# houkensjtu/taichi-2d-vof

Measured on AMD Instinct MI355X. Metric: cell-updates/sec (whole node), 4096x4096 fp64 dam-break, higher is better.
Workload: dtype f64; 1 GPU; 4096x4096 -ic 1 f64, dt 4e-06, 10 Jacobi sweeps/step, single strip; nx=4096, ny=4096, jacobi_iters=10, exchange=none, tm_choice=1, step_schedule=k_tm batch graphs (k_transport + the next step's k_momentum as one kernel), handle_warm_steps=19

## Files before the change

### taichi-2d-vof_amd/csrc/kernels/common.h

```cpp
#pragma once
#include "../vof2d_device.h"

namespace vof {

#ifdef VOF_WAVE_TIMES
__device__ unsigned long long* vof_wave_times = nullptr;
__device__ int vof_wave_kid = -1;
__device__ unsigned int vof_wave_cap = 0;
struct WaveTimer {
  unsigned long long t0, c0, wait;
  unsigned int wave;
  bool on;
  __device__ __forceinline__ WaveTimer(int kid) {
    on = vof_wave_times != nullptr && vof_wave_kid == kid;
    wave = blockIdx.x * (blockDim.x >> 6) + (threadIdx.x >> 6);
    t0 = on ? wall_clock64() : 0ull;
    c0 = on ? __builtin_readcyclecounter() : 0ull;
    wait = 0ull;
  }
  __device__ __forceinline__ void barrier() {
    if (on) {
      const unsigned long long t = __builtin_readcyclecounter();
      __syncthreads();
      wait += __builtin_readcyclecounter() - t;
    } else {
      __syncthreads();
    }
  }
  __device__ __forceinline__ ~WaveTimer() {
    if (on && (threadIdx.x & 63) == 0 && wave < vof_wave_cap) {
      vof_wave_times[2 * wave] = t0;
      vof_wave_times[2 * wave + 1] = wall_clock64();
      vof_wave_times[2 * vof_wave_cap + 2 * wave] = wait;
      vof_wave_times[2 * vof_wave_cap + 2 * wave + 1] = __builtin_readcyclecounter() - c0;
    }
  }
};
#else
struct WaveTimer {
  __device__ __forceinline__ WaveTimer(int) {}
  __device__ __forceinline__ void barrier() { __syncthreads(); }
};
#endif
#ifdef VOF_SHORTCUT_STATS
__device__ unsigned long long vof_stats[16];
#define VOF_STAT(k) do { if ((threadIdx.x & 63) == 0) atomicAdd(&vof::vof_stats[k], 1ull); } while (0)
#else
#define VOF_STAT(k) do { } while (0)
#endif
enum : int { WT_MOMENTUM = 0, WT_JACOBI_TB = 3, WT_FCT_X = 5, WT_FCT_Y = 6, WT_JACOBI = 2, WT_TRANSPORT = 12, WT_JACOBI_PAIR = 13, WT_TM = 14 };
enum : int {
  ABL_FIXED_ROW = 1,
  ABL_NO_STORE = 2,
  ABL_PRIO0 = 4,
  ABL_PRIO1 = 8,
  ABL_IDLE1 = 16,
  ABL_PASS0 = 32,
  ABL_NO_UPRED = 64,
  ABL_NO_VPRED = 128
};
template <typename T, int V>
struct Row {
  T l;
  T c[V];
  T r;
};

template <typename T, int V>
__device__ __forceinline__ void load_c(T (&c)[V], const T* __restrict__ p) {
  Pack<T, V> k = *reinterpret_cast<const Pack<T, V>*>(p);
#pragma unroll
  for (int q = 0; q < V; ++q) c[q] = k.v[q];
}
template <typename T, int V>
__device__ __forceinline__ void load_row(Row<T, V>& w, const T* __restrict__ p) {
  load_c<T, V>(w.c, p);
  w.l = p[-1];
  w.r = p[V];
}
template <typename T, int V>
__device__ __forceinline__ void load_c_nt(T (&c)[V], const T* __restrict__ p) {
  typedef T vec_t __attribute__((ext_vector_type(V)));
  vec_t k = __builtin_nontemporal_load(reinterpret_cast<const vec_t*>(p));
#pragma unroll
  for (int q = 0; q < V; ++q) c[q] = k[q];
}
template <typename T, int V>
__device__ __forceinline__ void store_c_nt(T* __restrict__ p, const T (&c)[V], int j0, int jlo, int jhi) {
  typedef T vec_t __attribute__((ext_vector_type(V)));
  if (j0 >= jlo && j0 + V - 1 <= jhi) {
    vec_t k;
#pragma unroll
    for (int q = 0; q < V; ++q) k[q] = c[q];
    __builtin_nontemporal_store(k, reinterpret_cast<vec_t*>(p));
  } else {
#pragma unroll
    for (int q = 0; q < V; ++q)
      if (j0 + q >= jlo && j0 + q <= jhi) p[q] = c[q];
  }
}
template <typename T, int V>
__device__ __forceinline__ void store_c(T* __restrict__ p, const T (&c)[V], int j0, int jlo, int jhi) {
  if (j0 >= jlo && j0 + V - 1 <= jhi) {
    Pack<T, V> k;
#pragma unroll
    for (int q = 0; q < V; ++q) k.v[q] = c[q];
    *reinterpret_cast<Pack<T, V>*>(p) = k;
  } else {
#pragma unroll
    for (int q = 0; q < V; ++q)
      if (j0 + q >= jlo && j0 + q <= jhi) p[q] = c[q];
  }
}
template <typename T, int V>
__device__ __forceinline__ void load_s(T (&c)[V], const T* __restrict__ p) { load_c_nt<T, V>(c, p); }
template <typename T, int V>
__device__ __forceinline__ void store_s(T* __restrict__ p, const T (&c)[V], int j0, int jlo, int jhi) {
  store_c_nt<T, V>(p, c, j0, jlo, jhi);
}
constexpr int kBufSkip = (int)0x80000000;
template <typename T>
__device__ __forceinline__ T* wave_uniform(T* p) {
  const unsigned long long v = (unsigned long long)p;
  const unsigned lo = __builtin_amdgcn_readfirstlane((unsigned)v), hi = __builtin_amdgcn_readfirstlane((unsigned)(v >> 32));
  return (T*)(((unsigned long long)hi << 32) | lo);
}
template <typename T, int V>
__device__ __forceinline__ void store_buf_nt(const T* base, int lane_off_bytes, int row_off_bytes, const T (&c)[V]) {
  static_assert(sizeof(T) * V == 16 || sizeof(T) * V == 8, "one b128 / b64 store per lane");
  row_off_bytes = __builtin_amdgcn_readfirstlane(row_off_bytes);
  lane_off_bytes += row_off_bytes;
  asm volatile("" : "+v"(lane_off_bytes));
  row_off_bytes = 0;
  const __amdgpu_buffer_rsrc_t r = __builtin_amdgcn_make_buffer_rsrc(wave_uniform(const_cast<T*>(base)), 0, kBufSkip, 0x00020000);
  typedef T vec_t __attribute__((ext_vector_type(V)));
  vec_t k;
#pragma unroll
  for (int q = 0; q < V; ++q) k[q] = c[q];
  if constexpr (sizeof(T) * V == 16) {
    typedef unsigned int u4 __attribute__((ext_vector_type(4)));
    __builtin_amdgcn_raw_buffer_store_b128(__builtin_bit_cast(u4, k), r, lane_off_bytes, row_off_bytes, 2 );
  } else {
    typedef unsigned int u2 __attribute__((ext_vector_type(2)));
    __builtin_amdgcn_raw_buffer_store_b64(__builtin_bit_cast(u2, k), r, lane_off_bytes, row_off_bytes, 2 );
  }
}
template <typename T, int V>
__device__ __forceinline__ void load_buf(T (&c)[V], const T* base, int lane_off_bytes, int row_off_bytes, bool nt) {
  static_assert(sizeof(T) * V == 16 || sizeof(T) * V == 8, "one b128 / b64 load per lane");
  row_off_bytes = __builtin_amdgcn_readfirstlane(row_off_bytes);
  const __amdgpu_buffer_rsrc_t r = __builtin_amdgcn_make_buffer_rsrc(wave_uniform(const_cast<T*>(base)), 0, kBufSkip, 0x00020000);
  typedef T vec_t __attribute__((ext_vector_type(V)));
  vec_t k;
  if constexpr (sizeof(T) * V == 16) {
    typedef unsigned int u4 __attribute__((ext_vector_type(4)));
    const u4 w = nt ? __builtin_amdgcn_raw_buffer_load_b128(r, lane_off_bytes, row_off_bytes, 2) : __builtin_amdgcn_raw_buffer_load_b128(r, lane_off_bytes, row_off_bytes, 0);
    k = __builtin_bit_cast(vec_t, w);
  } else {
    typedef unsigned int u2 __attribute__((ext_vector_type(2)));
    const u2 w = nt ? __builtin_amdgcn_raw_buffer_load_b64(r, lane_off_bytes, row_off_bytes, 2) : __builtin_amdgcn_raw_buffer_load_b64(r, lane_off_bytes, row_off_bytes, 0);
    k = __builtin_bit_cast(vec_t, w);
  }
#pragma unroll
  for (int q = 0; q < V; ++q) c[q] = k[q];
}
template <typename T, int V>
__device__ __forceinline__ T left_of(const Row<T, V>& w, int q) { return q == 0 ? w.l : w.c[q - 1]; }
template <typename T, int V>
__device__ __forceinline__ T right_of(const Row<T, V>& w, int q) { return q == V - 1 ? w.r : w.c[q + 1]; }

__device__ __forceinline__ int xcd_contiguous_block(int b, int n) {
  const int q = n >> 3, r = n & 7, x = b & 7;
  return x * q + (x < r ? x : r) + (b >> 3);
}
constexpr int kXcdGroup = 10;
__device__ __forceinline__ int xcd_grouped_block(int b, int n) {
  constexpr int WIN = 8 * kXcdGroup;
  const int base = (b / WIN) * WIN;
  if (base + WIN > n) return b;
  const int o = b - base;
  return base + (o & 7) * kXcdGroup + (o >> 3);
}

template <int V>
__device__ __forceinline__ bool wave_tile(const Geom& g, int first, int last, int R, int& j0, int& ra,
                                          int& rb) {
  const int wave = blockIdx.x * (blockDim.x >> 6) + __builtin_amdgcn_readfirstlane(threadIdx.x >> 6);
  const int lane = threadIdx.x & 63;
  const int tj = wave % g.ntj;
  const int ch = wave / g.ntj;
  j0 = 1 + tj * 64 * V + lane * V;
  ra = first + ch * R;
  rb = ra + R - 1 < last ? ra + R - 1 : last;
  return ra <= last && j0 <= g.ny;
}
__device__ __forceinline__ size_t at(const Geom& g, int i, int j) {
  return (size_t)(i - g.row_lo) * (size_t)g.pitch + (size_t)(g.col0 + j);
}

__device__ __forceinline__ int dpp_up(int v) { return __builtin_amdgcn_update_dpp(v, v, 0x138, 0xf, 0xf, false); }
__device__ __forceinline__ int dpp_dn(int v) { return __builtin_amdgcn_update_dpp(v, v, 0x130, 0xf, 0xf, false); }
__device__ __forceinline__ double lane_up(double x) {
  return __hiloint2double(dpp_up(__double2hiint(x)), dpp_up(__double2loint(x)));
}
__device__ __forceinline__ double lane_dn(double x) {
  return __hiloint2double(dpp_dn(__double2hiint(x)), dpp_dn(__double2loint(x)));
}
__device__ __forceinline__ float lane_up(float x) { return __int_as_float(dpp_up(__float_as_int(x))); }
__device__ __forceinline__ float lane_dn(float x) { return __int_as_float(dpp_dn(__float_as_int(x))); }
__device__ __forceinline__ int dpp_up_z(int v) { return __builtin_amdgcn_update_dpp(0, v, 0x138, 0xf, 0xf, true); }
__device__ __forceinline__ int dpp_dn_z(int v) { return __builtin_amdgcn_update_dpp(0, v, 0x130, 0xf, 0xf, true); }
__device__ __forceinline__ double lane_up_z(double x) {
  return __hiloint2double(dpp_up_z(__double2hiint(x)), dpp_up_z(__double2loint(x)));
}
__device__ __forceinline__ double lane_dn_z(double x) {
  return __hiloint2double(dpp_dn_z(__double2hiint(x)), dpp_dn_z(__double2loint(x)));
}
__device__ __forceinline__ float lane_up_z(float x) { return __int_as_float(dpp_up_z(__float_as_int(x))); }
__device__ __forceinline__ float lane_dn_z(float x) { return __int_as_float(dpp_dn_z(__float_as_int(x))); }

template <typename T> struct DivLimits;
template <> struct DivLimits<double> {
  static constexpr double lo = 1e-289, hi = 1e280, up = 0x1p+256, dn = 0x1p-256, qmin = 0x1p-766 ,
                          denorm_min = 0x1p-1074, half_step = 0x1p-819 ,
                          inf = __builtin_huge_val();
};
template <> struct DivLimits<float> {
  static constexpr float lo = 1e-25f, hi = 1e25f, up = 0x1p+96f, dn = 0x1p-96f, qmin = 0x1p-30f ,
                         denorm_min = 0x1p-149f, half_step = 0x1p-54f, inf = __builtin_huge_valf();
};
template <typename T> __device__ __forceinline__ T dfma(T a, T b, T c);
template <> __device__ __forceinline__ double dfma<double>(double a, double b, double c) { return __builtin_fma(a, b, c); }
template <> __device__ __forceinline__ float dfma<float>(float a, float b, float c) { return __builtin_fmaf(a, b, c); }

template <typename T>
__device__ __forceinline__ T div_scaled(T a, T b, T y, T scale) {
  const T A = a * scale;
  const T Q0 = A * y;
  return dfma<T>(dfma<T>(-b, Q0, A), y, Q0);
}

template <typename T>
__device__ __forceinline__ T div_tiny(T a, T b, T y) {
  using L = DivLimits<T>;
  const T A = a * L::up;
  const T Q = div_scaled<T>(a, b, y, L::up);
  T res = Q * L::dn;
  const T diff = dfma<T>(-res, L::up, Q);
  const T R = dfma<T>(-b, Q, A);
  const bool fix = dabs<T>(diff) == L::half_step && R != (T)0 && ((R > (T)0) == (b > (T)0)) == (diff > (T)0);
  const T adj = res + (diff > (T)0 ? L::denorm_min : -L::denorm_min);
  res = fix ? adj : res;
  return a != (T)0 ? res : a * y;
}

template <typename T, bool SMALL_B = false>
__device__ __forceinline__ T div_by_const(T a, T b, T y ) {
  using L = DivLimits<T>;
  const T q = a * y;
  const T r = dfma<T>(-b, q, a);
  T res = dfma<T>(r, y, q);
  const T aa = dabs<T>(a);
  if (aa < L::lo) {
    res = q;
    if (a != (T)0) res = div_tiny<T>(a, b, y);
  } else if (SMALL_B && aa > L::hi) {
    res = q;
    if (aa < L::inf) res = div_scaled<T>(a, b, y, L::dn) * L::up;
  }
  return res;
}

__device__ __forceinline__ bool tiny_nonzero(float a) {
  constexpr unsigned LO_BITS = __builtin_bit_cast(unsigned, DivLimits<float>::lo);
  return ((__float_as_uint(a) & 0x7fffffffu) - 1u) < (LO_BITS - 1u);
}

struct ColdFlag {
  int* p;
  __device__ __forceinline__ void operator()() const { if (p) *p = 1; }
};
struct ColdFlagLds {
  typedef __attribute__((address_space(3))) int lds_int;
  lds_int* p;
  __device__ __forceinline__ explicit ColdFlagLds(int* q) : p((lds_int*)q) {}
  __device__ __forceinline__ void operator()() const { *p = 1; }
};
template <typename T, int V, bool SMALL_B = false, typename Cold>
__device__ __forceinline__ void div_by_const_v(T (&res)[V], const T (&a)[V], const T (&b)[V], const T (&y)[V], const Cold& cold);
template <typename T, int V, bool SMALL_B = false>
__device__ __forceinline__ void div_by_const_v(T (&res)[V], const T (&a)[V], const T (&b)[V], const T (&y)[V],
                                               int* cold = nullptr ) {
  div_by_const_v<T, V, SMALL_B, ColdFlag>(res, a, b, y, ColdFlag{cold});
}
template <typename T, int V, bool SMALL_B, typename Cold>
__device__ __forceinline__ void div_by_const_v(T (&res)[V], const T (&a)[V], const T (&b)[V], const T (&y)[V], const Cold& cold) {
  bool odd = false;
  if constexpr (sizeof(T) == 4) {
#pragma unroll
    for (int q = 0; q < V; ++q) {
      const T q0 = a[q] * y[q];
      res[q] = dfma<T>(dfma<T>(-b[q], q0, a[q]), y[q], q0);
      odd = odd || tiny_nonzero(a[q]) || (SMALL_B && !(dabs<T>(a[q]) <= DivLimits<T>::hi));
    }
    if (odd) {
#pragma unroll
      for (int q = 0; q < V; ++q) {
        if constexpr (SMALL_B) res[q] = div_by_const<T, true>(a[q], b[q], y[q]);
        else {
          res[q] = dabs<T>(a[q]) < DivLimits<T>::lo ? div_tiny<T>(a[q], b[q], y[q]) : res[q];
          __builtin_amdgcn_sched_barrier(0);
        }
      }
      cold();
    }
  } else {
#pragma unroll
    for (int q = 0; q < V; ++q) {
      const T q0 = a[q] * y[q];
      res[q] = dfma<T>(dfma<T>(-b[q], q0, a[q]), y[q], q0);
      const T aa = dabs<T>(a[q]);
      odd = odd || !(aa >= DivLimits<T>::lo) || (SMALL_B && !(aa <= DivLimits<T>::hi));
    }
    if (odd) {
      bool nonzero = false;
#pragma unroll
      for (int q = 0; q < V; ++q) {
        const T aa = dabs<T>(a[q]);
        nonzero = nonzero || (a[q] != (T)0 && (!(aa >= DivLimits<T>::lo) || (SMALL_B && !(aa <= DivLimits<T>::hi))));
      }
      if (nonzero) {
#pragma unroll
        for (int q = 0; q < V; ++q) {
          if constexpr (SMALL_B) res[q] = div_by_const<T, true>(a[q], b[q], y[q]);
          else {
            res[q] = dabs<T>(a[q]) < DivLimits<T>::lo ? div_tiny<T>(a[q], b[q], y[q]) : res[q];
            __builtin_amdgcn_sched_barrier(0);
          }
        }
        cold();
      }
    }
  }
}
template <typename T>
__device__ __forceinline__ T div_by_const_inrange(T a, T b, T y) {
  const T q0 = a * y;
  return dfma<T>(dfma<T>(-b, q0, a), y, q0);
}

template <int N> struct IC { static constexpr int value = N; };

}
```

### taichi-2d-vof_amd/csrc/kernels/jacobi_pair.h

```cpp
#pragma once
#include "jacobi.h"

namespace vof {

template <typename T, int V>
struct JpRing {
  static constexpr int W = 64 * V, NR = 8;
  T p[NR][W], b[NR][W];
  int hit;
};
template <typename T, int V>
__device__ __forceinline__ void jp_put(T (&row)[64 * V], int lane, const T (&c)[V]) {
  Pack<T, V> k;
#pragma unroll
  for (int q = 0; q < V; ++q) k.v[q] = c[q];
  *reinterpret_cast<Pack<T, V>*>(&row[lane * V]) = k;
}
template <typename T, int V>
__device__ __forceinline__ void jp_get(T (&c)[V], const T (&row)[64 * V], int lane) {
  const Pack<T, V> k = *reinterpret_cast<const Pack<T, V>*>(&row[lane * V]);
#pragma unroll
  for (int q = 0; q < V; ++q) c[q] = k.v[q];
}

template <typename T, int V, int TS, bool BS, int ROLE, int ABL = 0>
__device__ __forceinline__ void jacobi_pair_march(const Geom& g, const Consts<T>& c, const T* __restrict__ p,
                                                  const T* __restrict__ rhs, T* __restrict__ pn, JpRing<T, V>& lds,
                                                  int c0, int lane, int ra, int rb, WaveTimer& wt) {
  if constexpr ((ROLE == 0 && !(ABL & ABL_PRIO0)) || (ROLE == 1 && (ABL & ABL_PRIO1))) __builtin_amdgcn_s_setprio(1);
  constexpr int W = 64 * V;
  constexpr int H = ((2 * TS + V - 1) / V) * V;
  const int j0 = c0 + lane * V;
  const int nx = g.nx, ny = g.ny;
  const int jlo = c0 + H > 1 ? c0 + H : 1;
  const int jhi = c0 + W - H - 1 < ny ? c0 + W - H - 1 : ny;
  const int64_t pitch = g.pitch;
  T cj[V], apI[V], yI[V];
#pragma unroll
  for (int q = 0; q < V; ++q) {
    const int j = j0 + q;
    const T an = j != ny ? c.dyi2 : (T)0.0, as_ = j != 1 ? c.dyi2 : (T)0.0;
    cj[q] = (j >= 1 && j <= ny) ? c.dxi2 : (T)0.0;
    apI[q] = (T)-1.0 * (c.dxi2 + c.dxi2 + an + as_);
    yI[q] = (T)1 / apI[q];
    if (j < 1 || j > ny) yI[q] = (T)0;
  }
  auto rowptr = [&](const T* base, int r) {
    if constexpr ((ABL & ABL_FIXED_ROW) != 0) r = ra;
    const int rc = r < g.row_lo ? g.row_lo : (r > g.row_hi ? g.row_hi : r);
    return base + (size_t)(rc - g.row_lo) * (size_t)pitch + (size_t)(g.col0 + j0);
  };
  auto to_products = [&](T (&row)[V], int r) {
    const bool rowok = r >= 1 && r <= nx;
#pragma unroll
    for (int q = 0; q < V; ++q) row[q] = (rowok ? cj[q] : (T)0.0) * row[q];
  };
  T ring[TS][3][V];
  T rq[6][V];
#pragma unroll
  for (int s = 0; s < TS; ++s)
#pragma unroll
    for (int k = 0; k < 3; ++k)
#pragma unroll
      for (int q = 0; q < V; ++q) ring[s][k][q] = (T)0;
#pragma unroll
  for (int k = 0; k < 6; ++k)
#pragma unroll
    for (int q = 0; q < V; ++q) rq[k][q] = (T)0;
  const int t0 = ra - TS + 2, t1 = rb + TS;
  if constexpr (ROLE == 0) {
    load_c<T, V>(ring[0][0], rowptr(p, t0 - 2));
    load_c<T, V>(ring[0][1], rowptr(p, t0 - 1));
    load_c<T, V>(ring[0][2], rowptr(p, t0));
    load_s<T, V>(rq[0], rowptr(rhs, t0 - 1));
  } else {
    for (int k = 0; k < 2 * TS + 2; ++k) wt.barrier();
    jp_get<T, V>(ring[0][0], lds.p[(t0 - 2) & 7], lane);
    jp_get<T, V>(ring[0][1], lds.p[(t0 - 1) & 7], lane);
    jp_get<T, V>(ring[0][2], lds.p[t0 & 7], lane);
    jp_get<T, V>(rq[0], lds.b[(t0 - 1) & 7], lane);
  }
  to_products(ring[0][0], t0 - 2);
  to_products(ring[0][1], t0 - 1);
  const T* const pn_tile = pn + (int64_t)(g.col0 + c0);
  const int voff_st = (j0 >= jlo && j0 + V - 1 <= jhi) ? lane * (int)(V * sizeof(T)) : kBufSkip;
  const T* const p_tile = p + (int64_t)(g.col0 + c0);
  const T* const rhs_tile = rhs + ((int64_t)(g.col0 + c0) - pitch);
  const int voff_ld = lane * (int)(V * sizeof(T));
  int soff = 0;
  auto sub = [&](auto uc, auto fc, int t) {
    constexpr int U = decltype(uc)::value;
    constexpr bool FAST = decltype(fc)::value != 0;
    constexpr int kM = U % 3, kC = (U + 1) % 3, kE = (U + 2) % 3;
    T carry[V];
    if constexpr (ROLE == 1 && (ABL & ABL_IDLE1)) { wt.barrier(); return; }
    if constexpr (ROLE == 0) jp_put<T, V>(lds.b[(t - 1) & 7], lane, rq[U % 6]);
    if constexpr (ROLE == 0 && (ABL & ABL_PASS0)) {
      const int io = t - TS;
      if (io >= ra && io <= rb) jp_put<T, V>(lds.p[io & 7], lane, ring[0][kC]);
      if (t < t1) {
        load_c<T, V>(ring[0][kM], rowptr(p, t + 1));
        load_s<T, V>(rq[(U + 1) % 6], rowptr(rhs, t));
      }
      wt.barrier();
      return;
    }
    if constexpr (FAST) {
#pragma unroll
      for (int q = 0; q < V; ++q) ring[0][kE][q] = cj[q] * ring[0][kE][q];
    } else {
      to_products(ring[0][kE], t);
    }
#pragma unroll
    for (int s = 1; s <= TS; ++s) {
      const int i = t - s;
      const T sl = lane_up_z(ring[s - 1][kC][V - 1]);
      const T sr = lane_dn_z(ring[s - 1][kC][0]);
      if (s > 1) {
        const T coef = (FAST || (i + 1 >= 1 && i + 1 <= nx)) ? c.dxi2 : (T)0.0;
#pragma unroll
        for (int q = 0; q < V; ++q) ring[s - 1][kE][q] = coef * carry[q];
      }
      if (!FAST && s > 1 && t < ra - TS + 2 * s) continue;
      const bool edge = !FAST && ((i == 1) || (i == nx));
      const int slot = ((U + 1 - s) % 6 + 6) % 6;
      T num[V];
#pragma unroll
      for (int q = 0; q < V; ++q) {
        const T N = q == V - 1 ? sr : ring[s - 1][kC][q + 1];
        const T S = q == 0 ? sl : ring[s - 1][kC][q - 1];
        num[q] = rq[slot][q] - ring[s - 1][kE][q] - ring[s - 1][kM][q] - N - S;
      }
      if (edge) {
        const T ae = i != nx ? c.dxi2 : (T)0.0;
        const T aw = i != 1 ? c.dxi2 : (T)0.0;
#pragma unroll
        for (int q = 0; q < V; ++q) {
          int j = j0 + q;
          asm volatile("" : "+v"(j));
          const T an = j != ny ? c.dyi2 : (T)0.0, as_ = j != 1 ? c.dyi2 : (T)0.0;
          const T ap = (T)-1.0 * (ae + aw + an + as_);
          T o = div_by_const<T>(num[q], ap, (T)1.0 / ap);
          if (j < 1 || j > ny) o = (T)0;
          carry[q] = o;
        }
      } else {
        div_by_const_v<T, V, false, ColdFlagLds>(carry, num, apI, yI, ColdFlagLds{&lds.hit});
      }
      if (s == 1) {
        if constexpr (FAST) {
          if constexpr (ROLE == 0) {
            load_buf<T, V>(ring[0][kM], p_tile, voff_ld, soff, false);
            load_buf<T, V>(rq[(U + 1) % 6], rhs_tile, voff_ld, soff, true);
            if constexpr ((ABL & ABL_FIXED_ROW) == 0) soff += (int)(pitch * (int64_t)sizeof(T));
          } else {
            jp_get<T, V>(ring[0][kM], lds.p[(t + 1) & 7], lane);
            jp_get<T, V>(rq[(U + 1) % 6], lds.b[t & 7], lane);
          }
        } else if (t < t1) {
          if constexpr (ROLE == 0) {
            load_c<T, V>(ring[0][kM], rowptr(p, t + 1));
            load_s<T, V>(rq[(U + 1) % 6], rowptr(rhs, t));
          } else {
            jp_get<T, V>(ring[0][kM], lds.p[(t + 1) & 7], lane);
            jp_get<T, V>(rq[(U + 1) % 6], lds.b[t & 7], lane);
          }
        }
      }
    }
    const int io = t - TS;
    if constexpr (ROLE == 0) {
      if (FAST || (io >= ra && io <= rb)) jp_put<T, V>(lds.p[io & 7], lane, carry);
    } else if constexpr ((ABL & ABL_NO_STORE) != 0) {
      asm volatile("" :: "v"(carry[0]), "v"(carry[V - 1]));
    } else if constexpr (BS) {
      if constexpr (FAST) {
        store_buf_nt<T, V>(pn_tile, voff_st, soff, carry);
        soff += (int)(pitch * (int64_t)sizeof(T));
      } else {
        store_buf_nt<T, V>(pn_tile, (io >= ra && io <= rb) ? voff_st : kBufSkip,
                           (io >= ra && io <= rb) ? (int)((int64_t)(io - g.row_lo) * pitch * (int64_t)sizeof(T)) : 0, carry);
      }
    } else if (FAST || (io >= ra && io <= rb)) {
      store_s<T, V>(pn + at(g, io, j0), carry, j0, jlo, jhi);
    }
    wt.barrier();
  };
  auto imax3 = [](int a, int b, int d) { return a > b ? (a > d ? a : d) : (b > d ? b : d); };
  auto imin3 = [](int a, int b, int d) { return a < b ? (a < d ? a : d) : (b < d ? b : d); };
  const int fast_lo = imax3(ra + TS, TS + 2, g.row_lo + TS);
  const int fast_hi = imin3(nx - 1, t1 - 1, g.row_hi - 1);
  int t = t0;
  bool done = false;
  for (int phase = 0; phase < 2; ++phase) {
    for (; !done && t <= t1 && (phase == 1 || t < fast_lo || t + 5 > fast_hi); t += 6) {
      sub(IC<0>{}, IC<0>{}, t);
      if (t + 1 > t1) { done = true; break; }
      sub(IC<1>{}, IC<0>{}, t + 1);
      if (t + 2 > t1) { done = true; break; }
      sub(IC<2>{}, IC<0>{}, t + 2);
      if (t + 3 > t1) { done = true; break; }
      sub(IC<3>{}, IC<0>{}, t + 3);
      if (t + 4 > t1) { done = true; break; }
      sub(IC<4>{}, IC<0>{}, t + 4);
      if (t + 5 > t1) { done = true; break; }
      sub(IC<5>{}, IC<0>{}, t + 5);
    }
    if (BS && phase == 0 && !done && t <= t1 && t >= fast_lo && t + 5 <= fast_hi) {
      soff = (int)((int64_t)((ROLE == 0 ? t + 1 : t - TS) - g.row_lo) * pitch * (int64_t)sizeof(T));
      for (; t + 5 <= fast_hi; t += 6) {
        sub(IC<0>{}, IC<1>{}, t);
        sub(IC<1>{}, IC<1>{}, t + 1);
        sub(IC<2>{}, IC<1>{}, t + 2);
        sub(IC<3>{}, IC<1>{}, t + 3);
        sub(IC<4>{}, IC<1>{}, t + 4);
        sub(IC<5>{}, IC<1>{}, t + 5);
      }
    }
  }
  if constexpr (ROLE == 0) { wt.barrier(); wt.barrier(); }
}

template <typename T, int V, int TS, bool BS, int ABL = 0>
__global__ __launch_bounds__(128) __attribute__((amdgpu_waves_per_eu(4))) void k_jacobi_pair(Geom g, Consts<T> c, const T* __restrict__ p,
                                                     const T* __restrict__ rhs, T* __restrict__ pn, int R, int ntt,
                                                     TbPlan tp, int first, int last) {
  constexpr int W = 64 * V;
  constexpr int H = ((2 * TS + V - 1) / V) * V;
  constexpr int STRIDE = W - 2 * H;
  __shared__ __attribute__((aligned(16))) JpRing<T, V> lds;
  WaveTimer wt_(WT_JACOBI_PAIR);
  if (last < first) { first = g.ilo; last = g.ihi; }
  const int pair = (int)blockIdx.x;
  const int role = __builtin_amdgcn_readfirstlane(threadIdx.x >> 6);
  const int lane = threadIdx.x & 63;
  int upair;
  upair = xcd_grouped_block(pair, (int)gridDim.x);
  int tj = upair % ntt, ra = first + (upair / ntt) * R, rb = ra + R - 1;
  bool planned = false;
  if (tp.masks != nullptr) {
    const unsigned long long* pl = tp.plan;
    if (pl[0] == plan_key(tp)) {
      const unsigned long long e = pl[1 + pair];
      tj = (int)(e & 0xffull);
      ra = (int)((e >> 8) & 0xfffffffull);
      rb = (int)((e >> 36) & 0xfffffffull);
      planned = true;
    }
  }
  tj = __builtin_amdgcn_readfirstlane(tj);
  ra = __builtin_amdgcn_readfirstlane(ra);
  rb = __builtin_amdgcn_readfirstlane(rb);
  if (planned && rb < ra) return;
  if (planned && ra < first) ra = first;
  if (ra > last) return;
  if (rb > last) rb = last;
  if (rb < ra) return;
  const int c0 = 1 - H + tj * STRIDE;
  if (threadIdx.x == 0) lds.hit = 0;
  __syncthreads();
  if (role == 0) {
    jacobi_pair_march<T, V, TS, BS, 0, ABL>(g, c, p, rhs, pn, lds, c0, lane, ra - TS, rb + TS, wt_);
  } else {
    jacobi_pair_march<T, V, TS, BS, 1, ABL>(g, c, p, rhs, pn, lds, c0, lane, ra, rb, wt_);
  }
  if (tp.masks != nullptr) {
    __syncthreads();
    if (threadIdx.x == 0 && lds.hit != 0) {
      for (int b = tb_band_of(g, ra < g.ilo ? g.ilo : ra); b <= tb_band_of(g, rb > g.ihi ? g.ihi : rb); ++b)
        atomicOr(tp.masks + tb_word(tp.par ^ 1, b, tj), 1ull << (tj & 63));
    }
  }
}

}
```

Before: 40.25 billion cell-updates/s.

## Stream Jacobi pair inputs via buffer-load-to-LDS DMA with lighter barriers

In the paired-wave Jacobi kernel, the producer wave's fast path now fetches the p and rhs rows directly into LDS ring slots using buffer_load_lds, prefetching D rows ahead and waiting on vmcnt, instead of loading them into registers and re-storing rhs to LDS. The per-row barrier becomes a raw s_barrier that waits only on LDS counters rather than the full __syncthreads. The aim is to hide global-memory latency and cut producer register/LDS traffic, at the cost of a larger LDS ring and a waves_per_eu hint lowered from 4 to 3 for fp64.

```diff
diff --git a/taichi-2d-vof_amd/csrc/kernels/common.h b/taichi-2d-vof_amd/csrc/kernels/common.h
--- a/taichi-2d-vof_amd/csrc/kernels/common.h
+++ b/taichi-2d-vof_amd/csrc/kernels/common.h
@@ -3,6 +3,12 @@
 
 namespace vof {
 
+__device__ __forceinline__ void lds_barrier_raw() {
+  asm volatile("" ::: "memory");
+  __builtin_amdgcn_s_waitcnt((15 << 0) | (7 << 4) | (0 << 8) | (3 << 14));
+  __builtin_amdgcn_s_barrier();
+  asm volatile("" ::: "memory");
+}
 #ifdef VOF_WAVE_TIMES
 __device__ unsigned long long* vof_wave_times = nullptr;
 __device__ int vof_wave_kid = -1;
@@ -27,6 +33,15 @@
       __syncthreads();
     }
   }
+  __device__ __forceinline__ void lds_barrier() {
+    if (on) {
+      const unsigned long long t = __builtin_readcyclecounter();
+      lds_barrier_raw();
+      wait += __builtin_readcyclecounter() - t;
+    } else {
+      lds_barrier_raw();
+    }
+  }
   __device__ __forceinline__ ~WaveTimer() {
     if (on && (threadIdx.x & 63) == 0 && wave < vof_wave_cap) {
       vof_wave_times[2 * wave] = t0;
@@ -40,6 +55,7 @@
 struct WaveTimer {
   __device__ __forceinline__ WaveTimer(int) {}
   __device__ __forceinline__ void barrier() { __syncthreads(); }
+  __device__ __forceinline__ void lds_barrier() { lds_barrier_raw(); }
 };
 #endif
 #ifdef VOF_SHORTCUT_STATS
diff --git a/taichi-2d-vof_amd/csrc/kernels/jacobi_pair.h b/taichi-2d-vof_amd/csrc/kernels/jacobi_pair.h
--- a/taichi-2d-vof_amd/csrc/kernels/jacobi_pair.h
+++ b/taichi-2d-vof_amd/csrc/kernels/jacobi_pair.h
@@ -3,12 +3,35 @@
 
 namespace vof {
 
-template <typename T, int V>
+#ifndef VOF_JP_DMA_D
+#define VOF_JP_DMA_D 3
+#endif
+template <typename T, int V, int TS, bool DMA>
 struct JpRing {
   static constexpr int W = 64 * V, NR = 8;
-  T p[NR][W], b[NR][W];
+  static constexpr int D = DMA ? VOF_JP_DMA_D : 1;
+  static constexpr int NB = DMA ? D + TS + 3 : 8;
+  static constexpr int NL = DMA ? D + 1 : 0;
+  static constexpr unsigned BIAS = 4096u * NB;
+  T p[NR][W], b[NB + NL][W];
   int hit;
+  __device__ __forceinline__ static int bslot(int r) { return DMA ? (int)((unsigned)(r + (int)BIAS) % (unsigned)NB) : (r & (NR - 1)); }
+  __device__ __forceinline__ static int lslot(int r) { return DMA ? NB + (int)((unsigned)(r + (int)BIAS) % (unsigned)NL) : 0; }
 };
+template <int N>
+__device__ __forceinline__ void wait_vmcnt() {
+  static_assert(N >= 0 && N < 64, "vmcnt is six bits");
+  asm volatile("" ::: "memory");
+  __builtin_amdgcn_s_waitcnt((N & 15) | (7 << 4) | (15 << 8) | ((N >> 4) << 14));
+  asm volatile("" ::: "memory");
+}
+template <bool NT, typename T>
+__device__ __forceinline__ void dma_row16(T* dst, const T* base, int lane_off_bytes, int row_off_bytes) {
+  row_off_bytes = __builtin_amdgcn_readfirstlane(row_off_bytes);
+  const __amdgpu_buffer_rsrc_t r = __builtin_amdgcn_make_buffer_rsrc(wave_uniform(const_cast<T*>(base)), 0, kBufSkip, 0x00020000);
+  __builtin_amdgcn_raw_ptr_buffer_load_lds(r, (__attribute__((address_space(3))) void*)dst, 16, lane_off_bytes, row_off_bytes, 0,
+                                           NT ? 2 : 0);
+}
 template <typename T, int V>
 __device__ __forceinline__ void jp_put(T (&row)[64 * V], int lane, const T (&c)[V]) {
   Pack<T, V> k;
@@ -23,10 +46,18 @@
   for (int q = 0; q < V; ++q) c[q] = k.v[q];
 }
 
+template <typename T, int V, bool BS, int ABL>
+constexpr bool jp_dma() { return BS && sizeof(T) * V == 16 && (ABL & ABL_PASS0) == 0; }
+
 template <typename T, int V, int TS, bool BS, int ROLE, int ABL = 0>
 __device__ __forceinline__ void jacobi_pair_march(const Geom& g, const Consts<T>& c, const T* __restrict__ p,
-                                                  const T* __restrict__ rhs, T* __restrict__ pn, JpRing<T, V>& lds,
+                                                  const T* __restrict__ rhs, T* __restrict__ pn,
+                                                  JpRing<T, V, TS, jp_dma<T, V, BS, ABL>()>& lds,
                                                   int c0, int lane, int ra, int rb, WaveTimer& wt) {
+  constexpr bool DMA = jp_dma<T, V, BS, ABL>();
+  using Ring = JpRing<T, V, TS, DMA>;
+  constexpr int D = Ring::D;
+  auto barrier = [&]() { if constexpr (DMA) wt.lds_barrier(); else wt.barrier(); };
   if constexpr ((ROLE == 0 && !(ABL & ABL_PRIO0)) || (ROLE == 1 && (ABL & ABL_PRIO1))) __builtin_amdgcn_s_setprio(1);
   constexpr int W = 64 * V;
   constexpr int H = ((2 * TS + V - 1) / V) * V;
@@ -74,11 +105,11 @@
     load_c<T, V>(ring[0][2], rowptr(p, t0));
     load_s<T, V>(rq[0], rowptr(rhs, t0 - 1));
   } else {
-    for (int k = 0; k < 2 * TS + 2; ++k) wt.barrier();
+    for (int k = 0; k < 2 * TS + 2; ++k) barrier();
     jp_get<T, V>(ring[0][0], lds.p[(t0 - 2) & 7], lane);
     jp_get<T, V>(ring[0][1], lds.p[(t0 - 1) & 7], lane);
     jp_get<T, V>(ring[0][2], lds.p[t0 & 7], lane);
-    jp_get<T, V>(rq[0], lds.b[(t0 - 1) & 7], lane);
+    jp_get<T, V>(rq[0], lds.b[Ring::bslot(t0 - 1)], lane);
   }
   to_products(ring[0][0], t0 - 2);
   to_products(ring[0][1], t0 - 1);
@@ -88,13 +119,22 @@
   const T* const rhs_tile = rhs + ((int64_t)(g.col0 + c0) - pitch);
   const int voff_ld = lane * (int)(V * sizeof(T));
   int soff = 0;
+  const int pitch_b = (int)(pitch * (int64_t)sizeof(T));
+  const int dma_lim = (g.row_hi - g.row_lo) * pitch_b;
+  auto dma_rows = [&](int r, int o) {
+    if constexpr (DMA) {
+      const int op = o + (D - 1) * pitch_b;
+      dma_row16<false>(&lds.b[Ring::lslot(r + D - 1)][0], p_tile, voff_ld, op < dma_lim ? op : dma_lim);
+      dma_row16<true>(&lds.b[Ring::bslot(r + D - 2)][0], rhs_tile, voff_ld, op < dma_lim + pitch_b ? op : dma_lim + pitch_b);
+    }
+  };
   auto sub = [&](auto uc, auto fc, int t) {
     constexpr int U = decltype(uc)::value;
     constexpr bool FAST = decltype(fc)::value != 0;
     constexpr int kM = U % 3, kC = (U + 1) % 3, kE = (U + 2) % 3;
     T carry[V];
-    if constexpr (ROLE == 1 && (ABL & ABL_IDLE1)) { wt.barrier(); return; }
-    if constexpr (ROLE == 0) jp_put<T, V>(lds.b[(t - 1) & 7], lane, rq[U % 6]);
+    if constexpr (ROLE == 1 && (ABL & ABL_IDLE1)) { barrier(); return; }
+    if constexpr (ROLE == 0 && !(DMA && FAST)) jp_put<T, V>(lds.b[Ring::bslot(t - 1)], lane, rq[U % 6]);
     if constexpr (ROLE == 0 && (ABL & ABL_PASS0)) {
       const int io = t - TS;
       if (io >= ra && io <= rb) jp_put<T, V>(lds.p[io & 7], lane, ring[0][kC]);
@@ -149,13 +189,19 @@
       }
       if (s == 1) {
         if constexpr (FAST) {
-          if constexpr (ROLE == 0) {
+          if constexpr (ROLE == 0 && DMA) {
+            dma_rows(t + 1, soff);
+            wait_vmcnt<2 * (D - 1)>();
+            jp_get<T, V>(ring[0][kM], lds.b[Ring::lslot(t + 1)], lane);
+            jp_get<T, V>(rq[(U + 1) % 6], lds.b[Ring::bslot(t)], lane);
+            if constexpr ((ABL & ABL_FIXED_ROW) == 0) soff += pitch_b;
+          } else if constexpr (ROLE == 0) {
             load_buf<T, V>(ring[0][kM], p_tile, voff_ld, soff, false);
             load_buf<T, V>(rq[(U + 1) % 6], rhs_tile, voff_ld, soff, true);
-            if constexpr ((ABL & ABL_FIXED_ROW) == 0) soff += (int)(pitch * (int64_t)sizeof(T));
+            if constexpr ((ABL & ABL_FIXED_ROW) == 0) soff += pitch_b;
           } else {
             jp_get<T, V>(ring[0][kM], lds.p[(t + 1) & 7], lane);
-            jp_get<T, V>(rq[(U + 1) % 6], lds.b[t & 7], lane);
+            jp_get<T, V>(rq[(U + 1) % 6], lds.b[Ring::bslot(t)], lane);
           }
         } else if (t < t1) {
           if constexpr (ROLE == 0) {
@@ -163,7 +209,7 @@
             load_s<T, V>(rq[(U + 1) % 6], rowptr(rhs, t));
           } else {
             jp_get<T, V>(ring[0][kM], lds.p[(t + 1) & 7], lane);
-            jp_get<T, V>(rq[(U + 1) % 6], lds.b[t & 7], lane);
+            jp_get<T, V>(rq[(U + 1) % 6], lds.b[Ring::bslot(t)], lane);
           }
         }
       }
@@ -176,7 +222,7 @@
     } else if constexpr (BS) {
       if constexpr (FAST) {
         store_buf_nt<T, V>(pn_tile, voff_st, soff, carry);
-        soff += (int)(pitch * (int64_t)sizeof(T));
+        soff += pitch_b;
       } else {
         store_buf_nt<T, V>(pn_tile, (io >= ra && io <= rb) ? voff_st : kBufSkip,
                            (io >= ra && io <= rb) ? (int)((int64_t)(io - g.row_lo) * pitch * (int64_t)sizeof(T)) : 0, carry);
@@ -184,7 +230,7 @@
     } else if (FAST || (io >= ra && io <= rb)) {
       store_s<T, V>(pn + at(g, io, j0), carry, j0, jlo, jhi);
     }
-    wt.barrier();
+    barrier();
   };
   auto imax3 = [](int a, int b, int d) { return a > b ? (a > d ? a : d) : (b > d ? b : d); };
   auto imin3 = [](int a, int b, int d) { return a < b ? (a < d ? a : d) : (b < d ? b : d); };
@@ -208,6 +254,11 @@
     }
     if (BS && phase == 0 && !done && t <= t1 && t >= fast_lo && t + 5 <= fast_hi) {
       soff = (int)((int64_t)((ROLE == 0 ? t + 1 : t - TS) - g.row_lo) * pitch * (int64_t)sizeof(T));
+      if constexpr (ROLE == 0 && DMA) {
+        jp_put<T, V>(lds.b[Ring::bslot(t - 1)], lane, rq[0]);
+#pragma unroll
+        for (int k = 0; k < D - 1; ++k) dma_rows(t + 2 - D + k, soff + (k + 1 - D) * pitch_b);
+      }
       for (; t + 5 <= fast_hi; t += 6) {
         sub(IC<0>{}, IC<1>{}, t);
         sub(IC<1>{}, IC<1>{}, t + 1);
@@ -216,19 +267,23 @@
         sub(IC<4>{}, IC<1>{}, t + 4);
         sub(IC<5>{}, IC<1>{}, t + 5);
       }
-    }
-  }
-  if constexpr (ROLE == 0) { wt.barrier(); wt.barrier(); }
-}
+      if constexpr (ROLE == 0 && DMA) wait_vmcnt<0>();
+    }
+  }
+  if constexpr (ROLE == 0) { barrier(); barrier(); }
+}
+
+template <typename T, int V, bool BS, int ABL>
+constexpr int jp_waves_per_eu() { return jp_dma<T, V, BS, ABL>() && sizeof(T) == 8 ? 3 : 4; }
 
 template <typename T, int V, int TS, bool BS, int ABL = 0>
-__global__ __launch_bounds__(128) __attribute__((amdgpu_waves_per_eu(4))) void k_jacobi_pair(Geom g, Consts<T> c, const T* __restrict__ p,
+__global__ __launch_bounds__(128) __attribute__((amdgpu_waves_per_eu(jp_waves_per_eu<T, V, BS, ABL>()))) void k_jacobi_pair(Geom g, Consts<T> c, const T* __restrict__ p,
                                                      const T* __restrict__ rhs, T* __restrict__ pn, int R, int ntt,
                                                      TbPlan tp, int first, int last) {
   constexpr int W = 64 * V;
   constexpr int H = ((2 * TS + V - 1) / V) * V;
   constexpr int STRIDE = W - 2 * H;
-  __shared__ __attribute__((aligned(16))) JpRing<T, V> lds;
+  __shared__ __attribute__((aligned(16))) JpRing<T, V, TS, jp_dma<T, V, BS, ABL>()> lds;
   WaveTimer wt_(WT_JACOBI_PAIR);
   if (last < first) { first = g.ilo; last = g.ihi; }
   const int pair = (int)blockIdx.x;
```

Measured after the change: 39.17 billion cell-updates/s, median of 2. 2.7% lower.
